# candrewlee14/zgml

Hardware: AMD Instinct MI355X
Metric: decode_tokens_per_sec (higher is better)
Workload: dtype f32; 1 GPU; SmolLM-135M Q4_0 greedy decode, batch 1, 1xMI355X (BASELINE configs[1]); weights=synthetic Q4_0 (int4 + f16 block scale / 32), tied f32 LM head, max_seq=2048, loop=device-resident (inputs in HBM), parallelism=none

## Files before the change

### zgml_amd/csrc/kernels.h

```cpp
#pragma once

#include <hip/hip_runtime.h>
#include <stdint.h>
#include <stdlib.h>

#include "../../include/zgml_hip.h"
#include "sample.h"
#include "switches.h"

namespace zgml {

inline uint32_t device_cus() {
    static const uint32_t n = [] {
        int dev = 0, cus = 0;
        if (hipGetDevice(&dev) != hipSuccess || hipDeviceGetAttribute(&cus, hipDeviceAttributeMultiprocessorCount, dev) != hipSuccess || cus <= 0) cus = 256;
        return (uint32_t)cus;
    }();
    return n;
}

constexpr int kMaxFusedSteps = 8;

struct FusedStepDev {
    uint32_t op;
// ... 278 lines not shown
void launch_attention_decode_batch(hipStream_t s, const AttnDecodeParams* dev_params, uint32_t n_heads, uint32_t d_head,
                                   const AttnSplit& sp, bool kvq = false);
void launch_kvq_attention_batch(hipStream_t s, const KvqAttentionParams* dev_params, uint32_t n_ops, uint32_t max_seq_q, uint32_t d_head,
                                const AttnSplit& sp = AttnSplit{});
bool attention_tiles_applies(uint32_t max_seq_q, uint32_t d_head);
struct AttnPieceSink {
    uint16_t* ap = nullptr;
    uint32_t S = 0, cols = 0;
};
void launch_attention_tiles(hipStream_t s, const AttentionParams* dev_params, uint32_t n_ops, uint32_t max_seq_q, uint32_t d_head,
                            const float* zero_word, const AttnPieceSink& sink = AttnPieceSink{});
enum class AttnRoute { generic, dense, rows, tiles };
AttnRoute attention_route(bool all_dense, uint32_t rows_d_head, uint32_t max_seq_q, const float* zero_word);
const char* attention_route_tag(AttnRoute r);
void launch_attention_batch(hipStream_t s, const AttentionParams* dev_params, uint32_t n_ops, uint32_t max_seq_q, bool all_dense,
                            uint32_t rows_d_head = 0, const float* zero_word = nullptr, const AttnPieceSink& sink = AttnPieceSink{});
struct DenseHeadTail;
void launch_dense_matmul(hipStream_t s, const DenseMatmulParams& p, DenseHeadTail* tail = nullptr);
struct ArgmaxAdvance {
    uint32_t* state = nullptr;
    int64_t* tokens = nullptr;
    uint32_t cap = 0;
    const float* embed = nullptr;
    float* tok_in = nullptr;
    uint32_t d = 0;
};
struct ResidentAhead;
void launch_argmax(hipStream_t s, const float* v, uint64_t n, float* scratch_val, int64_t* scratch_idx, int64_t* out,
                   const ArgmaxAdvance& adv = ArgmaxAdvance{}, const ResidentAhead* ahead = nullptr);
constexpr uint32_t kArgPairs = 1024;
void launch_argmax_fold(hipStream_t s, const float* scratch_val, const int64_t* scratch_idx, uint32_t nblk, int64_t* out, const ArgmaxAdvance& adv);
struct ResidentPrepArgs {
    const float *embed, *cos, *sin;
    float *tok_in, *mask;
    float* const* rope_bufs;
    const uint32_t *dyn_kind, *dyn_base, *dyn_stride;
    uint32_t* dyn;
    const uint32_t* state;
    const uint32_t* tokens;
    uint32_t d, max_seq, dh, n_rope, n_ops, T;
};
void launch_resident_prep(hipStream_t s, const ResidentPrepArgs& a, uint32_t total);
struct ResidentAhead {
    ResidentPrepArgs a;
    uint32_t total = 0;
};
struct DenseHeadTail {
    const float* logits = nullptr;
    uint32_t vocab = 0;
    float* pair_val = nullptr;
    int64_t* pair_idx = nullptr;
    ResidentAhead ahead;
    uint32_t pairs = 0;
};
struct ResidentBatchPrepArgs {
    const float *embed, *cos, *sin;
    float *tok_in, *mask;
    float* const* rope_bufs;
    const uint32_t *dyn_kind, *dyn_base, *dyn_stride, *dyn_seq;
    uint32_t* dyn;
    const uint32_t* state;
    uint32_t d, max_seq, dh, n_rope, n_ops, B;
};
void launch_resident_batch_prep(hipStream_t s, const ResidentBatchPrepArgs& a, uint32_t total);
int argmax_batch_blocks(uint64_t n);
void launch_argmax_batch(hipStream_t s, const float* v, uint64_t n, uint32_t B, float* scratch_val, int64_t* scratch_idx, uint32_t* state, int64_t* tokens);
void launch_argmax_rows_stage1(hipStream_t s, const float* v, uint64_t n, uint32_t rows, float* scratch_val, int64_t* scratch_idx);
enum SpecWord : uint32_t {
    kSpecTok = 0,
    kSpecPos,
    kSpecProduced,
    kSpecWanted,
    kSpecMode,
    kSpecNgram,
    kSpecNDrafts,
    kSpecStart,
    kSpecHistLo,
    kSpecSteps,
    kSpecDrafted,
    kSpecAccepted,
    kSpecRun,
    kSpecRunPos = kSpecRun + 1,
    kSpecWords = kSpecRun + 4,
};
struct SampleParamsDev;
struct SampleConstraintRow;
struct SpecArgs {
    uint32_t* words;
    uint32_t* hist;
    const uint32_t* drafts;
    uint32_t* cand;
    int64_t* tokens;
    const float* pval;
    const int64_t* pidx;
    uint32_t T, nblk, vocab, hist_cap, tokens_cap;
    const uint32_t* picks = nullptr;
    const SampleParamsDev* sparams = nullptr;
    const float* lp_rows = nullptr;
    float* lp_out = nullptr;
    const uint32_t* top_rows_tok = nullptr;
    const float* top_rows_val = nullptr;
    uint32_t* top_tok_out = nullptr;
    float* top_val_out = nullptr;
    const SampleConstraintRow* con_row = nullptr;
    uint32_t* con_state = nullptr;
    uint32_t* row_state = nullptr;
// ... 205 lines not shown
```

### zgml_amd/csrc/kernels_generic.hip

```cpp
#include "kernels.h"
#include <stdlib.h>

#include <hip/hip_fp16.h>
#include <math.h>

#include "attention_decode.h"
#include "tail_device.h"

namespace zgml {

namespace {

constexpr int kBlock = 256;

__device__ __forceinline__ float wave_sum(float v) {
#pragma unroll
    for (int off = 32; off > 0; off >>= 1) v += __shfl_xor(v, off, 64);
    return v;
}
__device__ __forceinline__ float wave_max(float v) {
#pragma unroll
    for (int off = 32; off > 0; off >>= 1) v = fmaxf(v, __shfl_xor(v, off, 64));
    return v;
}
// ... 164 lines not shown
                ((float4*)p.steps[s].store)[q] = make_float4(v[0], v[V > 1 ? 1 : 0], v[V > 2 ? 2 : 0], v[V > 3 ? 3 : 0]);
            else
                p.steps[s].store[q] = v[0];
        }
    }
    if (!p.ap) return;
    const uint32_t i = q * V, m = i / p.ap_cols, j = i - m * p.ap_cols;
    if (V == 1) {
        store_a_pieces(p.ap, p.ap_S, m, j, v[0]);
    } else if (p.ap_S & kApF16) {
        uint16_t h[4];
#pragma unroll
        for (int e = 0; e < 4; e++) h[e] = __half_as_ushort(__float2half_rn(v[e % V]));
        *(uint2*)(p.ap + a_f16_index(p.ap_S & ~kApF16, m, j)) = make_uint2(h[0] | ((uint32_t)h[1] << 16), h[2] | ((uint32_t)h[3] << 16));
    } else {
        uint32_t hp[4][kAPieces];
#pragma unroll
        for (int e = 0; e < 4; e++) split_a_pieces(v[e % V], hp[e]);
        uint16_t* const d = p.ap + a_piece_index(p.ap_S, m, j);
#pragma unroll
        for (int pc = 0; pc < kAPieces; pc++)
            *(uint2*)(d + 512 * pc) = make_uint2((hp[0][pc] >> 16) | (hp[1][pc] & 0xFFFF0000u), (hp[2][pc] >> 16) | (hp[3][pc] & 0xFFFF0000u));
    }
}

__global__ void __launch_bounds__(kBlock) layernorm_kernel(float* __restrict__ dst, const float* __restrict__ src,
                                                           uint32_t cols, float eps) {
    __shared__ float red[8];
    const float* s = src + (uint64_t)blockIdx.x * cols;
    float* d = dst + (uint64_t)blockIdx.x * cols;
    float mu = 0;
    for (uint32_t j = threadIdx.x; j < cols; j += kBlock) mu += s[j];
    mu = block_sum(mu, red) / (float)cols;
    float v = 0;
    for (uint32_t j = threadIdx.x; j < cols; j += kBlock) {
        float diff = s[j] - mu;
        v += diff * diff;
    }
    v = block_sum(v, red);
    float inv_std = 1.0f / sqrtf(v / (float)cols + eps);
    for (uint32_t j = threadIdx.x; j < cols; j += kBlock) d[j] = (s[j] - mu) * inv_std;
}

__global__ void __launch_bounds__(kBlock) rmsnorm_kernel(float* __restrict__ dst, const float* __restrict__ src,
                                                         uint32_t cols, float eps) {
    __shared__ float red[8];
    const float* s = src + (uint64_t)blockIdx.x * cols;
    float* d = dst + (uint64_t)blockIdx.x * cols;
    float ss = 0;
    for (uint32_t j = threadIdx.x; j < cols; j += kBlock) ss += s[j] * s[j];
    ss = block_sum(ss, red);
    float inv = 1.0f / sqrtf(ss / (float)cols + eps);
    for (uint32_t j = threadIdx.x; j < cols; j += kBlock) d[j] = s[j] * inv;
}

template <int NPT>
__global__ void __launch_bounds__(kBlock) row_chain_kernel(RowChainParams p) {
    __shared__ float red[8];
    const uint64_t base = (uint64_t)blockIdx.x * p.cols;
    const float* s = p.src + base;
    float* nd = p.norm_dst + base;
    float ss = 0;
    if (NPT > 0) {
        constexpr int N = NPT > 0 ? NPT : 1;
        __shared__ __attribute__((aligned(16))) uint16_t pl[kAPieces * N * kBlock];
        float v[N], mo[N];
        const uint32_t last = p.cols - 1;
        const uint32_t chunks = (p.cols + kBlock - 1) / kBlock;
        const uint32_t k_lo = blockIdx.y * chunks / gridDim.y, k_hi = (blockIdx.y + 1) * chunks / gridDim.y;
        if (p.add_dst) {
            const float *a0 = p.a0 + base, *a1 = p.a1 + base;
            float w[N];
#pragma unroll
            for (int k = 0; k < N; k++) v[k] = a0[min(threadIdx.x + k * kBlock, last)];
#pragma unroll
            for (int k = 0; k < N; k++) w[k] = a1[min(threadIdx.x + k * kBlock, last)];
#pragma unroll
            for (int k = 0; k < N; k++) v[k] = v[k] + w[k];
        } else {
#pragma unroll
            for (int k = 0; k < N; k++) v[k] = s[min(threadIdx.x + k * kBlock, last)];
        }
        if (p.mul_dst) {
#pragma unroll
            for (int k = 0; k < N; k++) mo[k] = p.mul_other[base + min(threadIdx.x + k * kBlock, last)];
        }
#pragma unroll
        for (int k = 0; k < N; k++) {
            const uint32_t j = threadIdx.x + k * kBlock;
            if (j < p.cols) {
                if (p.add_dst && (uint32_t)k >= k_lo && (uint32_t)k < k_hi) p.add_dst[base + j] = v[k];
                ss += v[k] * v[k];
            }
        }
        ss = block_sum(ss, red);
        const float inv = 1.0f / sqrtf(ss / (float)p.cols + p.eps);
#pragma unroll
        for (int k = 0; k < N; k++) {
            const uint32_t j = threadIdx.x + k * kBlock;
            if (j < p.cols && (uint32_t)k >= k_lo && (uint32_t)k < k_hi) {
                const float nv = v[k] * inv;
                nd[j] = nv;
                const float xv = p.mul_dst ? nv * mo[k] : nv;
                if (p.mul_dst) p.mul_dst[base + j] = xv;
                if (p.ap && (p.ap_S & kApF16)) {
                    pl[j] = __half_as_ushort(__float2half_rn(xv));
                } else if (p.ap) {
                    uint32_t hp[kAPieces];
                    split_a_pieces(xv, hp);
#pragma unroll
                    for (int pc = 0; pc < kAPieces; pc++) pl[pc * N * kBlock + j] = (uint16_t)(hp[pc] >> 16);
                }
            }
        }
        if (p.ap) {
            __syncthreads();
            const uint32_t c_lo = min(k_lo * kBlock, p.cols), c_hi = min(k_hi * kBlock, p.cols), groups = (c_hi - c_lo) / 8;
            const bool f16 = (p.ap_S & kApF16) != 0;
            for (uint32_t u = threadIdx.x; u < (f16 ? 1u : (uint32_t)kAPieces) * groups; u += kBlock) {
                const uint32_t piece = u / groups, j0 = c_lo + (u - piece * groups) * 8;
                const uint4 val = *(const uint4*)(pl + piece * (N * kBlock) + j0);
                uint16_t* const d = f16 ? p.ap + a_f16_index(p.ap_S & ~kApF16, blockIdx.x, j0) : p.ap + a_piece_index(p.ap_S, blockIdx.x, j0) + piece * 512;
                *(uint4*)d = val;
            }
        }
        return;
    }
    if (p.add_dst) {
        const float *a0 = p.a0 + base, *a1 = p.a1 + base;
        float* ad = p.add_dst + base;
        for (uint32_t j = threadIdx.x; j < p.cols; j += kBlock) {
            const float v = a0[j] + a1[j];
            ad[j] = v;
            ss += v * v;
        }
    } else {
        for (uint32_t j = threadIdx.x; j < p.cols; j += kBlock) ss += s[j] * s[j];
    }
    ss = block_sum(ss, red);
    const float inv = 1.0f / sqrtf(ss / (float)p.cols + p.eps);
    if (p.mul_dst) {
        const float* mo = p.mul_other + base;
        float* md = p.mul_dst + base;
        for (uint32_t j = threadIdx.x; j < p.cols; j += kBlock) {
            const float nv = s[j] * inv;
            nd[j] = nv;
            md[j] = nv * mo[j];
            if (p.ap) store_a_pieces(p.ap, p.ap_S, blockIdx.x, j, nv * mo[j]);
        }
// ... 598 lines not shown
    if (lane < LPK) {
        const float inv_l = r.l > 0.f ? 1.0f / r.l : 0.0f;
        *(float4*)(p.dst + (uint64_t)qi * p.dst_cs + 4 * lane) = make_float4(r.acc.x * inv_l, r.acc.y * inv_l, r.acc.z * inv_l, r.acc.w * inv_l);
    }
}


template <typename BT>
__global__ void __launch_bounds__(kBlock) dense_ncontig_kernel(DenseMatmulParams p) {
    uint32_t n = blockIdx.x * kBlock + threadIdx.x, m = blockIdx.y;
    if (n >= p.N) return;
    const float* a = p.a + (uint64_t)m * p.a_rs;
    const BT* b = (const BT*)p.b + n;
    float acc = 0.f;
    for (uint32_t k = 0; k < p.K; k++) acc = fmaf(a[(uint64_t)k * p.a_cs], (float)b[(uint64_t)k * p.b_rs], acc);
    p.dst[(uint64_t)m * p.dst_rs + n] = acc;
}

template <typename BT, int VEC>
__global__ void __launch_bounds__(kBlock) dense_kcontig_kernel(DenseMatmulParams p) {
    uint32_t n = blockIdx.x * (kBlock / 64) + (threadIdx.x >> 6), m = blockIdx.y;
    if (n >= p.N) return;
    uint32_t lane = threadIdx.x & 63;
    const float* a = p.a + (uint64_t)m * p.a_rs;
    const BT* b = (const BT*)p.b + (uint64_t)n * p.b_cs;
    float acc = 0.f;
    if (VEC == 4) {
        for (uint32_t k = lane * 4; k < p.K; k += 256) {
            float4 av = *(const float4*)(a + k);
            float b0, b1, b2, b3;
            if (sizeof(BT) == 4) {
                float4 bv = *(const float4*)((const float*)b + k);
                b0 = bv.x, b1 = bv.y, b2 = bv.z, b3 = bv.w;
            } else {
                const __half2* hp = (const __half2*)((const __half*)b + k);
                float2 lo = __half22float2(hp[0]), hi = __half22float2(hp[1]);
                b0 = lo.x, b1 = lo.y, b2 = hi.x, b3 = hi.y;
            }
            acc = fmaf(av.x, b0, acc);
            acc = fmaf(av.y, b1, acc);
            acc = fmaf(av.z, b2, acc);
            acc = fmaf(av.w, b3, acc);
        }
    } else {
        for (uint32_t k = lane; k < p.K; k += 64) acc = fmaf(a[(uint64_t)k * p.a_cs], (float)b[k], acc);
    }
    acc = wave_sum(acc);
    if (lane == 0) p.dst[(uint64_t)m * p.dst_rs + n] = acc;
}

constexpr uint32_t kStreamRows = 2, kStreamWgRows = kStreamRows * (kBlock / 64), kStreamMaxK = 1024, kStreamMaxWgs = 1024;
static_assert(kStreamMaxWgs <= kArgPairs, "one pair per workgroup of the streaming head must fit the argmax scratch");

template <int R, int KI>
__global__ void __launch_bounds__(kBlock) dense_kcontig_stream_kernel(DenseMatmulParams p, uint32_t head_wgs, float* pair_val, int64_t* pair_idx, ResidentAhead ahead) {
    if (blockIdx.x >= head_wgs) {
        resident_prep_ahead(ahead, (blockIdx.x - head_wgs) * kBlock + threadIdx.x);
        return;
    }
    const uint32_t lane = threadIdx.x & 63, wave = threadIdx.x >> 6;
    const float* const b = (const float*)p.b;
    uint32_t kc[KI];
    bool live[KI];
    float4 xv[KI];
#pragma unroll
    for (int it = 0; it < KI; it++) {
        const uint32_t k = lane * 4 + 256 * it;
        live[it] = k < p.K;
        kc[it] = live[it] ? k : 0;
        xv[it] = *(const float4*)(p.a + kc[it]);
    }
    float bv = -INFINITY;
    int64_t bi = INT64_MAX;
    for (uint64_t row0 = (uint64_t)blockIdx.x * (R * (kBlock / 64)) + wave * R; row0 < p.N; row0 += (uint64_t)head_wgs * (R * (kBlock / 64))) {
        float4 w[R][KI];
#pragma unroll
        for (int r = 0; r < R; r++) {
            const uint64_t n = row0 + r < p.N ? row0 + r : p.N - 1;
#pragma unroll
            for (int it = 0; it < KI; it++) w[r][it] = *(const float4*)(b + (uint64_t)n * p.b_cs + kc[it]);
        }
#pragma unroll
        for (int r = 0; r < R; r++) {
            float acc = 0.f;
#pragma unroll
            for (int it = 0; it < KI; it++) {
                float t = fmaf(xv[it].x, w[r][it].x, acc);
                t = fmaf(xv[it].y, w[r][it].y, t);
                t = fmaf(xv[it].z, w[r][it].z, t);
                t = fmaf(xv[it].w, w[r][it].w, t);
                acc = live[it] ? t : acc;
            }
            acc = wave_sum(acc);
            if (row0 + r < p.N) {
                if (lane == 0) p.dst[row0 + r] = acc;
                arg_fold(bv, bi, acc, (int64_t)(row0 + r));
            }
        }
    }
    if (!pair_val) return;
    __shared__ float sv[kBlock / 64];
    __shared__ int64_t si[kBlock / 64];
    if (lane == 0) sv[wave] = bv, si[wave] = bi;
    __syncthreads();
    if (threadIdx.x == 0) {
#pragma unroll
        for (int w2 = 1; w2 < kBlock / 64; w2++) arg_fold(bv, bi, sv[w2], si[w2]);
        pair_val[blockIdx.x] = bv, pair_idx[blockIdx.x] = bi;
    }
}

template <typename BT>
__global__ void __launch_bounds__(kBlock) dense_strided_kernel(DenseMatmulParams p) {
    uint32_t n = blockIdx.x * kBlock + threadIdx.x, m = blockIdx.y;
    if (n >= p.N) return;
    const float* a = p.a + (uint64_t)m * p.a_rs;
    const BT* b = (const BT*)p.b + (uint64_t)n * p.b_cs;
    float acc = 0.f;
    for (uint32_t k = 0; k < p.K; k++) acc = fmaf(a[(uint64_t)k * p.a_cs], (float)b[(uint64_t)k * p.b_rs], acc);
    p.dst[(uint64_t)m * p.dst_rs + n] = acc;
}

__global__ void __launch_bounds__(kBlock) copy_f4_kernel(float4* __restrict__ dst, const float4* __restrict__ src,
                                                         uint64_t n4) {
    for (uint64_t i = (uint64_t)blockIdx.x * kBlock + threadIdx.x; i < n4; i += (uint64_t)gridDim.x * kBlock)
        dst[i] = src[i];
}
template <int U, bool NT>
__global__ void __launch_bounds__(kBlock) copy_f4_unrolled_kernel(float4* __restrict__ dst, const float4* __restrict__ src, uint64_t n4) {
    typedef float f4v __attribute__((ext_vector_type(4)));
    const uint64_t stride = (uint64_t)gridDim.x * kBlock;
    uint64_t i = (uint64_t)blockIdx.x * kBlock + threadIdx.x;
    for (; i + (U - 1) * stride < n4; i += U * stride) {
        f4v v[U];
// ... 200 lines not shown
    switch (d_head) {
        case 8: ADEC(2, false); break;
        case 16: ADEC(4, false); break;
        case 32: ADEC(8, false); break;
        case 64: ADEC(16, false); break;
        case 128: ADEC(32, false); break;
        case 256: ADEC(64, false); break;
        default: break;
    }
#undef ADEC
}

void launch_attention_batch(hipStream_t s, const AttentionParams* dev_params, uint32_t n_ops, uint32_t max_seq_q,
                            bool all_dense, uint32_t rows_d_head, const float* zero_word, const AttnPieceSink& sink) {
    if (!n_ops || !max_seq_q) return;
    switch (attention_route(all_dense, rows_d_head, max_seq_q, zero_word)) {
        case AttnRoute::tiles: launch_attention_tiles(s, dev_params, n_ops, max_seq_q, rows_d_head, zero_word, sink); return;
        case AttnRoute::rows: {
            const dim3 grid(max_seq_q, n_ops);
            const uint32_t block = (uint64_t)max_seq_q * n_ops >= 256 ? 256 : kAttnBlock;
#define AROWS(L) attention_rows_kernel<L><<<grid, block, 0, s>>>(dev_params, zero_word)
            switch (rows_d_head) {
                case 8: AROWS(2); return;
                case 16: AROWS(4); return;
                case 32: AROWS(8); return;
                case 64: AROWS(16); return;
                case 128: AROWS(32); return;
                default: AROWS(64); return;
            }
#undef AROWS
        }
        case AttnRoute::dense: attention_dense_kernel<<<dim3(max_seq_q, n_ops), kAttnBlock, 0, s>>>(dev_params); return;
        case AttnRoute::generic: attention_kernel<<<dim3(max_seq_q, n_ops), kBlock, 0, s>>>(dev_params); return;
    }
}

AttnRoute attention_route(bool all_dense, uint32_t rows_d_head, uint32_t max_seq_q, const float* zero_word) {
    if (!all_dense) return AttnRoute::generic;
    const bool rows_dh = rows_d_head >= 8 && rows_d_head <= 256 && (rows_d_head & (rows_d_head - 1)) == 0;
    if (!(rows_dh && zero_word && sw().hip_attn_rows)) return AttnRoute::dense;
    return attention_tiles_applies(max_seq_q, rows_d_head) ? AttnRoute::tiles : AttnRoute::rows;
}

const char* attention_route_tag(AttnRoute r) {
    switch (r) {
        case AttnRoute::generic: return "attention-generic";
        case AttnRoute::dense: return "attention-dense";
        case AttnRoute::rows: return "attention-rows";
        case AttnRoute::tiles: return "attention-tiles";
    }
    return "attention";
}

static void launch_dense_kcontig_stream(hipStream_t s, const DenseMatmulParams& p, DenseHeadTail* tail) {
    constexpr int R = (int)kStreamRows;
    const uint32_t blocks = cdiv(p.N, kStreamWgRows), head_wgs = blocks < kStreamMaxWgs ? blocks : kStreamMaxWgs;
    const ResidentAhead ahead = tail ? tail->ahead : ResidentAhead{};
    float* const pv = tail ? tail->pair_val : nullptr;
    int64_t* const pi = tail ? tail->pair_idx : nullptr;
    const dim3 grid(head_wgs + cdiv(ahead.total, kBlock));
    switch (cdiv(p.K, 256)) {
        case 1: dense_kcontig_stream_kernel<R, 1><<<grid, kBlock, 0, s>>>(p, head_wgs, pv, pi, ahead); break;
        case 2: dense_kcontig_stream_kernel<R, 2><<<grid, kBlock, 0, s>>>(p, head_wgs, pv, pi, ahead); break;
        case 3: dense_kcontig_stream_kernel<R, 3><<<grid, kBlock, 0, s>>>(p, head_wgs, pv, pi, ahead); break;
        default: dense_kcontig_stream_kernel<R, 4><<<grid, kBlock, 0, s>>>(p, head_wgs, pv, pi, ahead); break;
    }
    if (pv) tail->pairs = head_wgs;
}

void launch_dense_matmul(hipStream_t s, const DenseMatmulParams& p, DenseHeadTail* tail) {
    if (p.M == 0 || p.N == 0) return;
    if (tail && (tail->logits != p.dst || tail->vocab != p.N)) tail = nullptr;
    const bool f16 = p.b_f16 != 0;
    if (p.b_cs == 1 && p.b_rs != 1) {
        dim3 grid(cdiv(p.N, kBlock), p.M);
        if (f16)
            dense_ncontig_kernel<__half><<<grid, kBlock, 0, s>>>(p);
        else
            dense_ncontig_kernel<float><<<grid, kBlock, 0, s>>>(p);
    } else if (p.b_rs == 1) {
        dim3 grid(cdiv(p.N, kBlock / 64), p.M);
        const uint32_t esz = f16 ? 2 : 4;
        bool vec = p.a_cs == 1 && (p.K % 4) == 0 && (p.a_rs % 4) == 0 && (p.b_cs % 4) == 0 &&
                   ((uintptr_t)p.a % 16) == 0 && ((uintptr_t)p.b % (4 * esz)) == 0;
        if (f16) {
            if (vec)
                dense_kcontig_kernel<__half, 4><<<grid, kBlock, 0, s>>>(p);
            else
                dense_kcontig_kernel<__half, 1><<<grid, kBlock, 0, s>>>(p);
        } else {
            if (vec && p.M == 1 && p.K <= kStreamMaxK)
                launch_dense_kcontig_stream(s, p, tail);
            else if (vec)
                dense_kcontig_kernel<float, 4><<<grid, kBlock, 0, s>>>(p);
            else
                dense_kcontig_kernel<float, 1><<<grid, kBlock, 0, s>>>(p);
        }
    } else {
        dim3 grid(cdiv(p.N, kBlock), p.M);
        if (f16)
            dense_strided_kernel<__half><<<grid, kBlock, 0, s>>>(p);
        else
            dense_strided_kernel<float><<<grid, kBlock, 0, s>>>(p);
    }
}

void launch_copy_f4(hipStream_t s, void* dst, const void* src, uint64_t bytes) {
    uint64_t n4 = bytes / 16;
    if (n4 == 0) return;
    const int variant = sw().copy_variant;
    if (variant == 0) {
        copy_f4_kernel<<<2048, kBlock, 0, s>>>((float4*)dst, (const float4*)src, n4);
        return;
    }
    if (variant == 1) {
        copy_f4_one_kernel<<<(unsigned)((n4 + kBlock - 1) / kBlock), kBlock, 0, s>>>((float4*)dst, (const float4*)src, n4);
        return;
    }
    if ((variant & 0xFF) == 3 || (variant & 0xFF) == 4) {
        const unsigned grid = (unsigned)(variant >> 8) ? (unsigned)(variant >> 8) : 688u;
        if ((variant & 0xFF) == 3)
            read_regions_kernel<false><<<grid, kBlock, 0, s>>>((float*)dst, (const float4*)src, n4);
        else
            read_regions_kernel<true><<<grid, kBlock, 0, s>>>((float*)dst, (const float4*)src, n4);
        return;
    }
    if (variant == 2) {
        read_f4_kernel<8><<<256 * 16, kBlock, 0, s>>>((float*)dst, (const float4*)src, n4);
        return;
    }
    const int U = variant & 0xFF, nt = (variant >> 8) & 1, bpc = (variant >> 16) & 0xFF ? (variant >> 16) & 0xFF : 8;
    const dim3 grid(256 * bpc);
    if (U >= 8)
        nt ? copy_f4_unrolled_kernel<8, true><<<grid, kBlock, 0, s>>>((float4*)dst, (const float4*)src, n4) : copy_f4_unrolled_kernel<8, false><<<grid, kBlock, 0, s>>>((float4*)dst, (const float4*)src, n4);
    else if (U >= 4)
        nt ? copy_f4_unrolled_kernel<4, true><<<grid, kBlock, 0, s>>>((float4*)dst, (const float4*)src, n4) : copy_f4_unrolled_kernel<4, false><<<grid, kBlock, 0, s>>>((float4*)dst, (const float4*)src, n4);
    else
        nt ? copy_f4_unrolled_kernel<2, true><<<grid, kBlock, 0, s>>>((float4*)dst, (const float4*)src, n4) : copy_f4_unrolled_kernel<2, false><<<grid, kBlock, 0, s>>>((float4*)dst, (const float4*)src, n4);
}

void launch_f32_to_f16(hipStream_t s, void* dst, const float* src, uint64_t n) {
    if (n == 0) return;
    f32_to_f16_kernel<<<1024, kBlock, 0, s>>>((__half*)dst, src, n);
}
// ... 3 lines not shown
```

### zgml_amd/csrc/runtime.hip

```cpp
#include "runtime_internal.h"

namespace zgml_rt {
std::string g_create_error;
}

namespace {


void fill_caps(zgml_capabilities* c) {
    memset(c, 0, sizeof(*c));
    c->compiled_programs = 1;
    c->host_visible_program_memory = 0;
    c->dense_matmul_f32 = 1;
    c->dense_matmul_f16 = 1;
    c->qmatmul = 1;
    c->fused_elementwise = 1;
    c->max_fused_elementwise_steps_has = 1;
    c->max_fused_elementwise_steps = kMaxFusedSteps;
    c->f16_weight_promotion = 1;
    c->dynamic_program_refresh = 1;
    c->prefill_attention = 1;
    c->decode_attention = 1;
    c->quantized_kv = 1;
    c->command_buffer_execution = 1;
// ... 306 lines not shown
bool same_static(const zgml_device_op& a, const zgml_device_op& b) {
    const size_t len = payload_bytes(a);
    if (a.kind != b.kind || !len) return false;
    const char *x = (const char*)&a.u, *y = (const char*)&b.u;
    size_t off = len, flen = 0;
    if (const DynField fa = dyn_field(a); fa.moves() && dyn_field(b).moves()) off = (size_t)((const char*)fa.word - x), flen = sizeof(uint32_t);
    if (a.kind == ZGML_DOP_FUSED_ELEMENTWISE) {
        const auto &fa = a.u.fused_elementwise, &fb = b.u.fused_elementwise;
        if (fa.n_steps != fb.n_steps) return false;
        for (uint32_t s = 0; s < fa.n_steps; s++)
            if (fa.steps[s].op != fb.steps[s].op || fa.steps[s].is_swapped != fb.steps[s].is_swapped ||
                fa.steps[s].secondary_buf != fb.steps[s].secondary_buf || fa.steps[s].secondary_offset != fb.steps[s].secondary_offset)
                return false;
        off = offsetof(zgml_op_fused_elementwise, steps), flen = sizeof(fa.steps);
    }
    return memcmp(x, y, off) == 0 && memcmp(x + off + flen, y + off + flen, len - off - flen) == 0;
}

}

namespace zgml_rt {

void set_dyn_from_ops(zgml_hip_program* p) {
    for (size_t i = 0; i < p->ops.size(); i++) {
        const DynField f = dyn_field(p->ops[i]);
        const uint32_t v = f.word ? *f.word : 0;
        if (p->dyn_host[i] != v) p->dyn_host[i] = v, p->dyn_dirty = true;
    }
}

void ensure_plan(zgml_hip_program* p) {
    if (p->plan_dirty || p->fuse_epoch != p->ctx->fuse_epoch) {
        free_graph(p);
        build_plan(p);
    }
}

bool capture_graph(zgml_hip_ctx* ctx, hipStream_t s, const char* tag, const std::function<void()>& work, hipGraph_t* g_out, hipGraphExec_t* e_out) {
    hipGraph_t g = nullptr;
    if (!CTX_CHECK(ctx, hipStreamBeginCapture(s, hipStreamCaptureModeThreadLocal))) return false;
    work();
    if (!CTX_CHECK(ctx, hipStreamEndCapture(s, &g)) || !g) return false;
    if (tag) dump_graph(g, tag);
    hipGraphExec_t ge = nullptr;
    if (!CTX_CHECK(ctx, hipGraphInstantiate(&ge, g, nullptr, nullptr, 0))) {
        hipGraphDestroy(g);
        return false;
    }
    *g_out = g, *e_out = ge;
    return true;
}

void run_plan(zgml_hip_program* p, hipStream_t s, size_t first, size_t count, DenseHeadTail* tail) {
    const auto run = [&](Launch& L) { tail && L.run_tail && &L == &p->plan.back() ? L.run_tail(s, tail) : L.run(s); };
#ifdef ZGML_TRACE
    static unsigned mod_period = 0, mod_mask = 0;
    static bool mod_init = false;
    if (!mod_init) {
        mod_init = true;
        if (const char* e = sw().hip_skip_mod) sscanf(e, "%u:%x", &mod_period, &mod_mask);
    }
    for (size_t i = first; i < first + count && i < p->plan.size(); i++) {
        if (sw().hip_skip_kinds & (1u << p->plan[i].kind)) continue;
        if (mod_period && i >= 1 && (mod_mask & (1u << ((i - 1) % mod_period)))) continue;
        run(p->plan[i]);
    }
#else
    for (size_t i = first; i < first + count && i < p->plan.size(); i++) run(p->plan[i]);
#endif
}

void flush_dyn(zgml_hip_program* p) {
    if (!p->dyn_dirty || p->ops.empty()) return;
    hipMemcpyAsync(p->dyn_dev, p->dyn_host, p->ops.size() * sizeof(uint32_t), hipMemcpyHostToDevice, p->ctx->stream);
    p->dyn_dirty = false;
}

void enqueue(zgml_hip_program* p) {
    zgml_hip_ctx* ctx = p->ctx;
    ensure_plan(p);
    flush_dyn(p);
    if (ctx->opt_profile) {
        hipEvent_t e0, e1;
        hipEventCreate(&e0);
        hipEventCreate(&e1);
        for (auto& L : p->plan) {
            hipEventRecord(e0, ctx->stream);
            L.run(ctx->stream);
            hipEventRecord(e1, ctx->stream);
            hipEventSynchronize(e1);
            float ms = 0;
            hipEventElapsedTime(&ms, e0, e1);
            if (L.kind < ZGML_DOP_COUNT) p->profile.time_ns[L.kind] += (uint64_t)(ms * 1e6);
            L.prof_ns += (uint64_t)(ms * 1e6);
            L.prof_calls++;
        }
        hipEventDestroy(e0);
        hipEventDestroy(e1);
        if (sw().hip_debug_plan.value >= 2 && p->plan[0].prof_calls == 8) {
            for (size_t i = 0; i < p->plan.size() && i < 40; i++)
                fprintf(stderr, "[zgml_hip] launch %3zu kind %2u ops %4u [%u..%u]  %.2f us\n", i, p->plan[i].kind, p->plan[i].n_ops,
                        p->plan[i].op_lo, p->plan[i].op_hi, p->plan[i].prof_ns / 1e3 / p->plan[i].prof_calls);
        }
        return;
    }
    if (ctx->opt_graph && !p->plan.empty()) {
        if (!p->graph_exec) {
            const int split_env = sw().hip_graph_split;
            size_t head = p->plan.size() >= 48 ? std::max<size_t>(8, p->plan.size() / 6) : p->plan.size();
            if (split_env == 0) head = p->plan.size();
            if (split_env > 0) head = std::min<size_t>((size_t)split_env, p->plan.size());
            auto capture = [&](size_t first, size_t count, hipGraph_t* g_out, hipGraphExec_t* e_out, const char* tag) {
                return capture_graph(ctx, ctx->stream, tag, [&] { run_plan(p, ctx->stream, first, count); }, g_out, e_out);
            };
            if (capture(0, head, &p->graph, &p->graph_exec, "program") && head < p->plan.size() &&
                !capture(head, p->plan.size() - head, &p->graph_tail, &p->graph_tail_exec, "program-tail")) {
                hipGraphExecDestroy(p->graph_exec), hipGraphDestroy(p->graph);
                p->graph_exec = nullptr, p->graph = nullptr;
            }
        }
        if (p->graph_exec) {
            CTX_CHECK(ctx, hipGraphLaunch(p->graph_exec, ctx->stream));
// ... 1053 lines not shown
```

### zgml_amd/csrc/runtime_internal.h

```cpp
#pragma once
#include <hip/hip_runtime.h>

#include <algorithm>
#include <chrono>
#include <cstdio>
#include <cstdlib>
#include <cstring>
#include <functional>
#include <map>
#include <memory>
#include <string>
#include <vector>

#include "kernels.h"
#include "schedule.h"

using namespace zgml;

namespace zgml_rt {

extern std::string g_create_error;

struct SplitHook {
    const float* out = nullptr;
// ... 199 lines not shown
    void* stage_dev = nullptr;
    uint64_t stage_cap = 0;
    void* stage_out_host = nullptr;
    hipGraph_t io_graph = nullptr;
    hipGraphExec_t io_graph_exec = nullptr;
    uint32_t io_in_rows = 0, io_out_rows = 0;
    bool pin_allowed = false;
    void* pin_host = nullptr;
    void* pin_dev = nullptr;
    uint64_t pin_size = 0;
    const void* pin_cand = nullptr;
    uint32_t pin_seen = 0;
    bool pin_off = false;
    void* io_out_dev = nullptr;
    IoPlan in_plan, out_plan;
    uint64_t staged_bytes = 0, staged_n = 0;
    zgml_runtime_profile profile{};
    zgml_resident* resident = nullptr;
    std::vector<zgml_shard_point> shard_points;
    uint16_t shard_logits_buf = 0;
    uint64_t shard_vocab = 0;
    hipGraph_t shard_graph = nullptr;
    hipGraphExec_t shard_graph_exec = nullptr;
    bool shard_capture_failed = false;
    std::vector<double> shard_point_us;
    bool shard_pair_argmax = false;
    unsigned long long* shard_pairs = nullptr;
    struct ShardPeer* shard_peer = nullptr;
};

#define CTX_CHECK(ctx, expr) (ctx)->check((expr), #expr)

namespace {
inline hipError_t h2d_sync(hipStream_t s, void* dst, const void* src, size_t bytes) {
    const hipError_t e = hipMemcpyAsync(dst, src, bytes, hipMemcpyHostToDevice, s);
    return e != hipSuccess ? e : hipStreamSynchronize(s);
}
inline hipError_t memset_sync(hipStream_t s, void* dst, int value, size_t bytes) {
    const hipError_t e = hipMemsetAsync(dst, value, bytes, s);
    return e != hipSuccess ? e : hipStreamSynchronize(s);
}
}

namespace zgml_rt {
void build_plan(zgml_hip_program* p);
void free_param_blobs(zgml_hip_program* p);
void free_graph(zgml_hip_program* p);
void dump_graph(hipGraph_t g, const char* tag);
void ensure_plan(zgml_hip_program* p);
bool capture_graph(zgml_hip_ctx* ctx, hipStream_t s, const char* tag, const std::function<void()>& work, hipGraph_t* g_out, hipGraphExec_t* e_out);
void set_dyn_from_ops(zgml_hip_program* p);
void flush_dyn(zgml_hip_program* p);
void run_plan(zgml_hip_program* p, hipStream_t s, size_t first, size_t count, DenseHeadTail* tail = nullptr);
void enqueue(zgml_hip_program* p);
void unhoist_if_guarded(zgml_hip_program* p, uint16_t buf_idx);
void free_kv_move_pool(zgml_hip_ctx* ctx);
void free_resident_graph(zgml_hip_program* p);
void free_resident(zgml_hip_program* p);
bool has_constraint(const zgml_hip_program* p);
}
```

### zgml_amd/csrc/runtime_resident.hip

```cpp
#include "runtime_internal.h"
#include "sample.h"
#include "sample_params.h"
#include "spec.h"

enum SampledKind { kKindPick, kKindLogprobs, kKindTop, kSampledKinds };
constexpr uint32_t kSampledForms = kSampledSels * kSampledKinds;
constexpr uint32_t sampled_form(uint32_t sel, uint32_t kind) { return kind * kSampledSels + sel; }
static const char* const kSampledFormNames[kSampledForms] = {"sampled", "penalized", "constrained", "constrained_rows",
                                                             "sampled_logprobs", "penalized_logprobs", "constrained_logprobs", "constrained_rows_logprobs",
                                                             "sampled_top", "penalized_top", "constrained_top", "constrained_rows_top"};

struct zgml_hip_constraint;
struct zgml_resident {
    float *embed = nullptr, *cos = nullptr, *sin = nullptr;
    uint32_t vocab = 0, d = 0, max_seq = 0, dh = 0, n_rope = 0;
    float *tok_in = nullptr, *mask = nullptr, *logits = nullptr;
    float** rope_bufs = nullptr;
    uint32_t* dyn_kind = nullptr;
    uint32_t* dyn_base = nullptr;
    uint32_t* dyn_stride = nullptr;
    uint32_t* state = nullptr;
    uint32_t token_len = 1;
    uint32_t* tok_dev = nullptr;
    int64_t* tokens = nullptr;
// ... 544 lines not shown
              CTX_CHECK(ctx, h2d_sync(ctx->stream, r->embed, d->token_embed, emb)) &&
              CTX_CHECK(ctx, h2d_sync(ctx->stream, r->cos, d->cos_table, tab)) &&
              CTX_CHECK(ctx, h2d_sync(ctx->stream, r->sin, d->sin_table, tab)) &&
              CTX_CHECK(ctx, h2d_sync(ctx->stream, r->rope_bufs, ropes.data(), ropes.size() * sizeof(float*))) &&
              CTX_CHECK(ctx, h2d_sync(ctx->stream, r->dyn_kind, kind.data(), n_ops * 4)) &&
              CTX_CHECK(ctx, h2d_sync(ctx->stream, r->dyn_base, base.data(), n_ops * 4)) &&
              CTX_CHECK(ctx, h2d_sync(ctx->stream, r->dyn_stride, stride.data(), n_ops * 4));
    if (ok && r->n_seqs) {
        std::vector<uint32_t> seq(n_ops + 1, 0);
        for (size_t i = 0; i < n_ops; i++) seq[i] = kind[i] && i < p->op_seq.size() && p->op_seq[i] != UINT32_MAX ? p->op_seq[i] : 0;
        const size_t pairs = (size_t)T * argmax_batch_blocks(d->vocab);
        ok = CTX_CHECK(ctx, hipMalloc((void**)&r->bstate, ((size_t)4 * r->n_seqs + 1) * 4)) && CTX_CHECK(ctx, hipMalloc((void**)&r->dyn_seq, (n_ops + 1) * 4)) &&
             CTX_CHECK(ctx, hipMalloc((void**)&r->bval, pairs * sizeof(float))) && CTX_CHECK(ctx, hipMalloc((void**)&r->bidx, pairs * sizeof(int64_t))) &&
             CTX_CHECK(ctx, h2d_sync(ctx->stream, r->dyn_seq, seq.data(), n_ops * 4));
    }
    if (!ok) {
        free_resident(p);
        return -1;
    }
    unhoist_if_guarded(p, d->buf_token_input);
    unhoist_if_guarded(p, d->buf_attn_mask);
    for (uint32_t l = 0; l < d->n_rope; l++) unhoist_if_guarded(p, d->buf_rope[l]);
    return 0;
}

int zgml_hip_resident_decode(zgml_hip_ctx* ctx, zgml_hip_program* p, uint32_t first_token, uint32_t start_pos,
                             uint32_t n_steps, int64_t* tokens_out) {
    if (!ctx || !p || !p->resident || !tokens_out) return -1;
    Resident* r = p->resident;
    if (refuse_constrained(ctx, p, "resident_decode")) return -1;
    if (r->n_seqs) {
        ctx->fail("resident_decode: the program is a batched plan (sequences declared: use zgml_hip_resident_decode_batch)");
        return -1;
    }
    if (r->token_len != 1) {
        ctx->fail("resident_decode: the program is a token_len > 1 plan (use zgml_hip_resident_prefill)");
        return -1;
    }
    if (first_token >= r->vocab || (uint64_t)start_pos + n_steps > r->max_seq) {
        ctx->fail("resident_decode: token or position out of range");
        return -1;
    }
    hipSetDevice(ctx->device);
    hipStream_t s = ctx->stream;
    resident_begin(p, [&] {
        return !n_steps || (positions_in_bounds(p, 1, [&](uint32_t) { return start_pos; }) && positions_in_bounds(p, 1, [&](uint32_t) { return start_pos + n_steps - 1; }));
    });
    if (!ensure_tokens(ctx, p, r->tokens, r->tokens_cap, n_steps)) return -1;
    const Prep prep = prep_args(p, r->state, r->state );
    const ArgmaxAdvance adv{r->state, r->tokens, r->tokens_cap, r->embed, r->tok_in, r->d};
    DenseHeadTail head;
    head.logits = r->logits, head.vocab = r->vocab, head.pair_val = ctx->arg_val, head.pair_idx = ctx->arg_idx;
    head.ahead = ResidentAhead{prep.a, prep.total - r->token_len * r->d};
    auto one_token = [&](hipStream_t st) {
        head.pairs = 0;
        run_plan(p, st, 0, p->plan.size(), &head);
        if (head.pairs)
            launch_argmax_fold(st, ctx->arg_val, ctx->arg_idx, head.pairs, ctx->arg_out, adv);
        else
            launch_argmax(st, r->logits, r->vocab, ctx->arg_val, ctx->arg_idx, ctx->arg_out, adv, &head.ahead);
        r->tail_launches = head.pairs ? 1 : 2;
    };
    const uint32_t st0[4] = {first_token, start_pos, 0, 0};
    if (!CTX_CHECK(ctx, hipMemcpyAsync(r->state, st0, sizeof(st0), hipMemcpyHostToDevice, s))) return -1;
    if (n_steps) launch_resident_prep(s, prep.a, prep.total);
    capture_once(ctx, s, "resident", false, one_token, &r->graph, &r->graph_exec);
    const uint32_t per_graph = (uint32_t)sw().hip_resident_tokens_per_graph;
    const auto tokens_of_a_graph = [&] {
        for (uint32_t t = 0; t < per_graph; t++) one_token(s);
    };
    if (ctx->opt_graph && r->graph_exec && per_graph > 1 && n_steps >= per_graph && !r->graph_multi_exec &&
        capture_graph(ctx, s, nullptr, tokens_of_a_graph, &r->graph_multi, &r->graph_multi_exec))
        r->multi_n = per_graph;
    for (uint32_t i = 0; i < n_steps;) {
        if (r->graph_multi_exec && n_steps - i >= r->multi_n) {
            hipGraphLaunch(r->graph_multi_exec, s);
            i += r->multi_n;
        } else if (r->graph_exec) {
            hipGraphLaunch(r->graph_exec, s);
            i++;
        } else {
            one_token(s);
            i++;
        }
    }
    hipMemcpyAsync(tokens_out, r->tokens, (size_t)n_steps * 8, hipMemcpyDeviceToHost, s);
    bool ok = CTX_CHECK(ctx, hipStreamSynchronize(s));
    ok = ok && ctx->handoff_ok("resident_decode");
    resident_end(p, n_steps, p->plan.size() + r->tail_launches);
    return ok ? 0 : -1;
}


int zgml_hip_resident_decode_batch(zgml_hip_ctx* ctx, zgml_hip_program* p, const uint32_t* first_tokens, const uint32_t* start_pos,
                                   const uint32_t* n_steps, uint32_t max_steps, int64_t* tokens_out) {
    if (!ctx || !p) return -1;
    Resident* r = p->resident;
    if (!r || !r->n_seqs || !p->n_seqs) {
        ctx->fail("resident_decode_batch: not a batched program with a resident set-up (zgml_hip_program_set_sequences, then zgml_hip_resident_setup)");
        return -1;
    }
    if (refuse_verify_plan(ctx, r, "resident_decode_batch")) return -1;
    if (!first_tokens || !start_pos || !n_steps || (max_steps && !tokens_out)) return -1;
    if (refuse_constrained(ctx, p, "resident_decode_batch")) return -1;
    const uint32_t B = r->n_seqs;
    uint32_t steps = 0;
    std::vector<uint32_t> last_pos;
    if (!batch_request(ctx, r, "resident_decode_batch", first_tokens, start_pos, n_steps, max_steps, tokens_out, nullptr, &steps, &last_pos)) return -1;
    if (!steps) return 0;
    hipSetDevice(ctx->device);
    hipStream_t s = ctx->stream;
    resident_begin(p, [&] {
        return positions_in_bounds(p, 1, [&](uint32_t i) { return start_pos[p->op_seq[i]]; }) && positions_in_bounds(p, 1, [&](uint32_t i) { return last_pos[p->op_seq[i]]; });
    });
    if (!ensure_tokens(ctx, p, r->btokens, r->btokens_cap, (uint64_t)B * steps)) return -1;
    const BatchPrep prep = batch_prep_args(p);
    auto one_step = [&](hipStream_t st) {
        launch_resident_batch_prep(st, prep.a, prep.total);
        run_plan(p, st, 0, p->plan.size());
        launch_argmax_batch(st, r->logits, r->vocab, B, r->bval, r->bidx, r->bstate, r->btokens);
    };
    std::vector<uint32_t> st0((size_t)4 * B + 1, 0);
    for (uint32_t b = 0; b < B; b++) st0[b] = first_tokens[b], st0[B + b] = start_pos[b], st0[2 * B + b] = n_steps[b];
    st0[4 * B] = steps;
    if (!CTX_CHECK(ctx, hipMemcpyAsync(r->bstate, st0.data(), st0.size() * 4, hipMemcpyHostToDevice, s)) ||
        !CTX_CHECK(ctx, hipMemsetAsync(r->btokens, 0xFF, (size_t)B * steps * 8, s)))
        return -1;
    capture_once(ctx, s, "resident_batch", true, one_step, &r->graph, &r->graph_exec);
    replay(s, r->graph_exec, steps, one_step);
    std::vector<int64_t> got((size_t)B * steps);
    hipMemcpyAsync(got.data(), r->btokens, got.size() * 8, hipMemcpyDeviceToHost, s);
    bool ok = CTX_CHECK(ctx, hipStreamSynchronize(s));
    ok = ok && ctx->handoff_ok("resident_decode_batch");
    for (uint32_t b = 0; ok && b < B; b++)
        for (uint32_t i = 0; i < steps; i++) tokens_out[(uint64_t)b * max_steps + i] = got[(uint64_t)b * steps + i];
    resident_end(p, steps, p->plan.size() + 3);
    return ok ? 0 : -1;
}



int64_t zgml_hip_sample(zgml_hip_ctx* ctx, zgml_hip_program* p, uint16_t buf_idx, uint64_t offset, uint64_t n, const zgml_sampling* sampling,
// ... 760 lines not shown
```

Measured before the change: 1686 tokens/s.

## Fuse final RMSNorm row-chain into the streaming LM-head kernel

After: 1695 tokens/s, median of 6. No clear change (+0.5%).

```diff
diff --git a/zgml_amd/csrc/kernels.h b/zgml_amd/csrc/kernels.h
--- a/zgml_amd/csrc/kernels.h
+++ b/zgml_amd/csrc/kernels.h
@@ -354,6 +354,8 @@
     int64_t* pair_idx = nullptr;
     ResidentAhead ahead;
     uint32_t pairs = 0;
+    const RowChainParams* norm = nullptr;
+    bool probe = false, norm_taken = false;
 };
 struct ResidentBatchPrepArgs {
     const float *embed, *cos, *sin;
diff --git a/zgml_amd/csrc/kernels_generic.hip b/zgml_amd/csrc/kernels_generic.hip
--- a/zgml_amd/csrc/kernels_generic.hip
+++ b/zgml_amd/csrc/kernels_generic.hip
@@ -240,6 +240,16 @@
     ss = block_sum(ss, red);
     float inv = 1.0f / sqrtf(ss / (float)cols + eps);
     for (uint32_t j = threadIdx.x; j < cols; j += kBlock) d[j] = s[j] * inv;
+}
+
+template <int N>
+__device__ __forceinline__ float row_chain_inv_rms(const float (&v)[N], uint32_t cols, float eps, float* red) {
+    float ss = 0;
+#pragma unroll
+    for (int k = 0; k < N; k++)
+        if (threadIdx.x + k * kBlock < cols) ss += v[k] * v[k];
+    ss = block_sum(ss, red);
+    return 1.0f / sqrtf(ss / (float)cols + eps);
 }
 
 template <int NPT>
@@ -276,13 +286,9 @@
 #pragma unroll
         for (int k = 0; k < N; k++) {
             const uint32_t j = threadIdx.x + k * kBlock;
-            if (j < p.cols) {
-                if (p.add_dst && (uint32_t)k >= k_lo && (uint32_t)k < k_hi) p.add_dst[base + j] = v[k];
-                ss += v[k] * v[k];
-            }
-        }
-        ss = block_sum(ss, red);
-        const float inv = 1.0f / sqrtf(ss / (float)p.cols + p.eps);
+            if (j < p.cols && p.add_dst && (uint32_t)k >= k_lo && (uint32_t)k < k_hi) p.add_dst[base + j] = v[k];
+        }
+        const float inv = row_chain_inv_rms(v, p.cols, p.eps, red);
 #pragma unroll
         for (int k = 0; k < N; k++) {
             const uint32_t j = threadIdx.x + k * kBlock;
@@ -987,12 +993,20 @@
 constexpr uint32_t kStreamRows = 2, kStreamWgRows = kStreamRows * (kBlock / 64), kStreamMaxK = 1024, kStreamMaxWgs = 1024;
 static_assert(kStreamMaxWgs <= kArgPairs, "one pair per workgroup of the streaming head must fit the argmax scratch");
 
-template <int R, int KI>
-__global__ void __launch_bounds__(kBlock) dense_kcontig_stream_kernel(DenseMatmulParams p, uint32_t head_wgs, float* pair_val, int64_t* pair_idx, ResidentAhead ahead) {
+struct HeadNormArgs {
+    const float *src = nullptr, *gain = nullptr;
+    float *norm_dst = nullptr, *mul_dst = nullptr;
+    float eps = 0.f;
+};
+constexpr int kHeadNormNpt = (int)kStreamMaxK / kBlock;
+
+template <int R, int KI, bool NORM>
+__global__ void __launch_bounds__(kBlock) dense_kcontig_stream_kernel(DenseMatmulParams p, uint32_t head_wgs, float* pair_val, int64_t* pair_idx, ResidentAhead ahead, HeadNormArgs nrm) {
     if (blockIdx.x >= head_wgs) {
         resident_prep_ahead(ahead, (blockIdx.x - head_wgs) * kBlock + threadIdx.x);
         return;
     }
+    if (NORM) __builtin_amdgcn_s_waitcnt(0);
     const uint32_t lane = threadIdx.x & 63, wave = threadIdx.x >> 6;
     const float* const b = (const float*)p.b;
     uint32_t kc[KI];
@@ -1003,18 +1017,46 @@
         const uint32_t k = lane * 4 + 256 * it;
         live[it] = k < p.K;
         kc[it] = live[it] ? k : 0;
-        xv[it] = *(const float4*)(p.a + kc[it]);
+        xv[it] = *(const float4*)((NORM ? nrm.src : p.a) + kc[it]);
+    }
+    float4 w[R][KI];
+    const auto load_rows = [&](uint64_t r0) {
+#pragma unroll
+        for (int r = 0; r < R; r++) {
+            const uint64_t n = r0 + r < p.N ? r0 + r : p.N - 1;
+#pragma unroll
+            for (int it = 0; it < KI; it++) w[r][it] = *(const float4*)(b + (uint64_t)n * p.b_cs + kc[it]);
+        }
+    };
+    uint64_t row0 = (uint64_t)blockIdx.x * (R * (kBlock / 64)) + wave * R;
+    bool loaded = false;
+    if (NORM) {
+        __shared__ float red[8];
+        float rv[kHeadNormNpt];
+        float4 gv[KI];
+#pragma unroll
+        for (int k = 0; k < kHeadNormNpt; k++) rv[k] = nrm.src[min(threadIdx.x + k * kBlock, p.K - 1)];
+#pragma unroll
+        for (int it = 0; it < KI; it++) gv[it] = *(const float4*)(nrm.gain + kc[it]);
+        load_rows(row0);
+        loaded = true;
+        const float inv = row_chain_inv_rms(rv, p.K, nrm.eps, red);
+        const bool stores = blockIdx.x == 0 && wave == 0;
+#pragma unroll
+        for (int it = 0; it < KI; it++) {
+            const float4 nv = make_float4(xv[it].x * inv, xv[it].y * inv, xv[it].z * inv, xv[it].w * inv);
+            xv[it] = make_float4(nv.x * gv[it].x, nv.y * gv[it].y, nv.z * gv[it].z, nv.w * gv[it].w);
+            if (stores && live[it]) {
+                *(float4*)(nrm.norm_dst + kc[it]) = nv;
+                *(float4*)(nrm.mul_dst + kc[it]) = xv[it];
+            }
+        }
     }
     float bv = -INFINITY;
     int64_t bi = INT64_MAX;
-    for (uint64_t row0 = (uint64_t)blockIdx.x * (R * (kBlock / 64)) + wave * R; row0 < p.N; row0 += (uint64_t)head_wgs * (R * (kBlock / 64))) {
-        float4 w[R][KI];
-#pragma unroll
-        for (int r = 0; r < R; r++) {
-            const uint64_t n = row0 + r < p.N ? row0 + r : p.N - 1;
-#pragma unroll
-            for (int it = 0; it < KI; it++) w[r][it] = *(const float4*)(b + (uint64_t)n * p.b_cs + kc[it]);
-        }
+    for (; row0 < p.N; row0 += (uint64_t)head_wgs * (R * (kBlock / 64))) {
+        if (!loaded) load_rows(row0);
+        loaded = false;
 #pragma unroll
         for (int r = 0; r < R; r++) {
             float acc = 0.f;
@@ -1321,6 +1363,20 @@
     return "attention";
 }
 
+static bool head_carries_norm(const DenseMatmulParams& p, const RowChainParams& rc) {
+    if (rc.add_dst || rc.ap || !rc.src || !rc.norm_dst || !rc.mul_dst || !rc.mul_other) return false;
+    if (rc.mul_dst != p.a || rc.cols != p.K || (p.K % 4) != 0 || p.K > kStreamMaxK) return false;
+    for (const float* q : {rc.src, rc.mul_other, (const float*)rc.norm_dst, (const float*)rc.mul_dst})
+        if ((uintptr_t)q % 16) return false;
+    const auto meet = [](const float* a, uint64_t na, const float* b, uint64_t nb) { return a < b + nb && b < a + na; };
+    const uint64_t K = p.K;
+    for (const float* w : {(const float*)rc.norm_dst, (const float*)rc.mul_dst})
+        if (meet(w, K, rc.src, K) || meet(w, K, rc.mul_other, K) || meet(w, K, p.dst, p.N) ||
+            meet(w, K, (const float*)p.b, (uint64_t)(p.N - 1) * p.b_cs + K))
+            return false;
+    return !meet(rc.norm_dst, K, rc.mul_dst, K);
+}
+
 static void launch_dense_kcontig_stream(hipStream_t s, const DenseMatmulParams& p, DenseHeadTail* tail) {
     constexpr int R = (int)kStreamRows;
     const uint32_t blocks = cdiv(p.N, kStreamWgRows), head_wgs = blocks < kStreamMaxWgs ? blocks : kStreamMaxWgs;
@@ -1328,19 +1384,42 @@
     float* const pv = tail ? tail->pair_val : nullptr;
     int64_t* const pi = tail ? tail->pair_idx : nullptr;
     const dim3 grid(head_wgs + cdiv(ahead.total, kBlock));
+    if (pv && tail->norm && head_carries_norm(p, *tail->norm)) {
+        const RowChainParams& rc = *tail->norm;
+        const HeadNormArgs nrm{rc.src, rc.mul_other, rc.norm_dst, rc.mul_dst, rc.eps};
+        switch (cdiv(p.K, 256)) {
+            case 1: dense_kcontig_stream_kernel<R, 1, true><<<grid, kBlock, 0, s>>>(p, head_wgs, pv, pi, ahead, nrm); break;
+            case 2: dense_kcontig_stream_kernel<R, 2, true><<<grid, kBlock, 0, s>>>(p, head_wgs, pv, pi, ahead, nrm); break;
+            case 3: dense_kcontig_stream_kernel<R, 3, true><<<grid, kBlock, 0, s>>>(p, head_wgs, pv, pi, ahead, nrm); break;
+            default: dense_kcontig_stream_kernel<R, 4, true><<<grid, kBlock, 0, s>>>(p, head_wgs, pv, pi, ahead, nrm); break;
+        }
+        tail->pairs = head_wgs;
+        return;
+    }
+    const HeadNormArgs none{};
     switch (cdiv(p.K, 256)) {
-        case 1: dense_kcontig_stream_kernel<R, 1><<<grid, kBlock, 0, s>>>(p, head_wgs, pv, pi, ahead); break;
-        case 2: dense_kcontig_stream_kernel<R, 2><<<grid, kBlock, 0, s>>>(p, head_wgs, pv, pi, ahead); break;
-        case 3: dense_kcontig_stream_kernel<R, 3><<<grid, kBlock, 0, s>>>(p, head_wgs, pv, pi, ahead); break;
-        default: dense_kcontig_stream_kernel<R, 4><<<grid, kBlock, 0, s>>>(p, head_wgs, pv, pi, ahead); break;
+        case 1: dense_kcontig_stream_kernel<R, 1, false><<<grid, kBlock, 0, s>>>(p, head_wgs, pv, pi, ahead, none); break;
+        case 2: dense_kcontig_stream_kernel<R, 2, false><<<grid, kBlock, 0, s>>>(p, head_wgs, pv, pi, ahead, none); break;
+        case 3: dense_kcontig_stream_kernel<R, 3, false><<<grid, kBlock, 0, s>>>(p, head_wgs, pv, pi, ahead, none); break;
+        default: dense_kcontig_stream_kernel<R, 4, false><<<grid, kBlock, 0, s>>>(p, head_wgs, pv, pi, ahead, none); break;
     }
     if (pv) tail->pairs = head_wgs;
 }
 
 void launch_dense_matmul(hipStream_t s, const DenseMatmulParams& p, DenseHeadTail* tail) {
+    DenseHeadTail* const asked = tail && tail->probe ? tail : nullptr;
+    if (asked) asked->norm_taken = false;
     if (p.M == 0 || p.N == 0) return;
     if (tail && (tail->logits != p.dst || tail->vocab != p.N)) tail = nullptr;
     const bool f16 = p.b_f16 != 0;
+    const uint32_t esz = f16 ? 2 : 4;
+    const bool vec = p.a_cs == 1 && (p.K % 4) == 0 && (p.a_rs % 4) == 0 && (p.b_cs % 4) == 0 &&
+                     ((uintptr_t)p.a % 16) == 0 && ((uintptr_t)p.b % (4 * esz)) == 0;
+    const bool stream = p.b_rs == 1 && !f16 && vec && p.M == 1 && p.K <= kStreamMaxK;
+    if (asked) {
+        asked->norm_taken = stream && tail && tail->pair_val && tail->norm && head_carries_norm(p, *tail->norm);
+        return;
+    }
     if (p.b_cs == 1 && p.b_rs != 1) {
         dim3 grid(cdiv(p.N, kBlock), p.M);
         if (f16)
@@ -1349,16 +1428,13 @@
             dense_ncontig_kernel<float><<<grid, kBlock, 0, s>>>(p);
     } else if (p.b_rs == 1) {
         dim3 grid(cdiv(p.N, kBlock / 64), p.M);
-        const uint32_t esz = f16 ? 2 : 4;
-        bool vec = p.a_cs == 1 && (p.K % 4) == 0 && (p.a_rs % 4) == 0 && (p.b_cs % 4) == 0 &&
-                   ((uintptr_t)p.a % 16) == 0 && ((uintptr_t)p.b % (4 * esz)) == 0;
         if (f16) {
             if (vec)
                 dense_kcontig_kernel<__half, 4><<<grid, kBlock, 0, s>>>(p);
             else
                 dense_kcontig_kernel<__half, 1><<<grid, kBlock, 0, s>>>(p);
         } else {
-            if (vec && p.M == 1 && p.K <= kStreamMaxK)
+            if (stream)
                 launch_dense_kcontig_stream(s, p, tail);
             else if (vec)
                 dense_kcontig_kernel<float, 4><<<grid, kBlock, 0, s>>>(p);
diff --git a/zgml_amd/csrc/runtime.hip b/zgml_amd/csrc/runtime.hip
--- a/zgml_amd/csrc/runtime.hip
+++ b/zgml_amd/csrc/runtime.hip
@@ -382,7 +382,10 @@
 }
 
 void run_plan(zgml_hip_program* p, hipStream_t s, size_t first, size_t count, DenseHeadTail* tail) {
-    const auto run = [&](Launch& L) { tail && L.run_tail && &L == &p->plan.back() ? L.run_tail(s, tail) : L.run(s); };
+    const auto run = [&](Launch& L) {
+        if (tail && tail->norm_taken && &L + 1 == &p->plan.back()) return;
+        tail && L.run_tail && &L == &p->plan.back() ? L.run_tail(s, tail) : L.run(s);
+    };
 #ifdef ZGML_TRACE
     static unsigned mod_period = 0, mod_mask = 0;
     static bool mod_init = false;
@@ -398,6 +401,21 @@
 #else
     for (size_t i = first; i < first + count && i < p->plan.size(); i++) run(p->plan[i]);
 #endif
+}
+
+bool head_takes_final_norm(zgml_hip_program* p, DenseHeadTail* tail) {
+    tail->norm = nullptr, tail->norm_taken = false;
+    const size_t n = p->plan.size();
+    if (n < 2 || !p->plan[n - 1].run_tail || !p->plan[n - 2].rc_desc || p->plan[n - 2].rc_rows != 1) return false;
+    const Launch &chain = p->plan[n - 2], &head = p->plan[n - 1];
+    for (uint64_t b : p->barriers)
+        if (b > std::min(chain.op_lo, head.op_lo) && b <= std::max(chain.op_hi, head.op_hi)) return false;
+    tail->norm = p->plan[n - 2].rc_desc.get();
+    tail->probe = true;
+    p->plan[n - 1].run_tail(nullptr, tail);
+    tail->probe = false;
+    if (!tail->norm_taken) tail->norm = nullptr;
+    return tail->norm_taken;
 }
 
 void flush_dyn(zgml_hip_program* p) {
diff --git a/zgml_amd/csrc/runtime_internal.h b/zgml_amd/csrc/runtime_internal.h
--- a/zgml_amd/csrc/runtime_internal.h
+++ b/zgml_amd/csrc/runtime_internal.h
@@ -275,6 +275,7 @@
 void set_dyn_from_ops(zgml_hip_program* p);
 void flush_dyn(zgml_hip_program* p);
 void run_plan(zgml_hip_program* p, hipStream_t s, size_t first, size_t count, DenseHeadTail* tail = nullptr);
+bool head_takes_final_norm(zgml_hip_program* p, DenseHeadTail* tail);
 void enqueue(zgml_hip_program* p);
 void unhoist_if_guarded(zgml_hip_program* p, uint16_t buf_idx);
 void free_kv_move_pool(zgml_hip_ctx* ctx);
diff --git a/zgml_amd/csrc/runtime_resident.hip b/zgml_amd/csrc/runtime_resident.hip
--- a/zgml_amd/csrc/runtime_resident.hip
+++ b/zgml_amd/csrc/runtime_resident.hip
@@ -620,6 +620,7 @@
     DenseHeadTail head;
     head.logits = r->logits, head.vocab = r->vocab, head.pair_val = ctx->arg_val, head.pair_idx = ctx->arg_idx;
     head.ahead = ResidentAhead{prep.a, prep.total - r->token_len * r->d};
+    const size_t plan_launches = p->plan.size() - (head_takes_final_norm(p, &head) ? 1 : 0);
     auto one_token = [&](hipStream_t st) {
         head.pairs = 0;
         run_plan(p, st, 0, p->plan.size(), &head);
@@ -655,7 +656,7 @@
     hipMemcpyAsync(tokens_out, r->tokens, (size_t)n_steps * 8, hipMemcpyDeviceToHost, s);
     bool ok = CTX_CHECK(ctx, hipStreamSynchronize(s));
     ok = ok && ctx->handoff_ok("resident_decode");
-    resident_end(p, n_steps, p->plan.size() + r->tail_launches);
+    resident_end(p, n_steps, plan_launches + r->tail_launches);
     return ok ? 0 : -1;
 }
 
```
